# pjmikkol/bwtc

Measured on AMD Instinct MI355X. Metric: MB/s compressed (BWT+encode) on 256 MiB block, higher is better.
Workload: dtype u8/u32/u64 integer

## Files before the change

### bwtc_amd/csrc/bwt_engine.hip

```cpp
#include "bwt_engine.hpp"
#include "radix_sort.hpp"
#include <algorithm>
#include <cmath>
#include <cstdlib>
#include <cstring>
#include <chrono>
#include <ctime>
#include <sys/prctl.h>

namespace bwtc_hip {

constexpr int kLoadTPB = 256;
constexpr int kLoadTile = kLoadTPB * 16;
constexpr u32 kTextPad = 128;

__global__ __launch_bounds__(kLoadTPB) void k_load_hist(const u8* __restrict__ src,
                                                        u8* __restrict__ T, u32 ncopy,
                                                        u32 padded, int reverse, int aligned,
                                                        u32* __restrict__ freqs) {
  __shared__ __attribute__((aligned(16))) u8 s_src[kLoadTile + 48];
  __shared__ u32 s_hist[256 * 16];
  const u32 tid = threadIdx.x;
  for (u32 i = tid; i < 256 * 16; i += kLoadTPB) s_hist[i] = 0;
  const u32 ntiles = (padded + (u32)kLoadTile - 1u) / (u32)kLoadTile;
// ... 462 lines not shown
      else { const u64 full = (fc << need) | ((x_hi << 32) | x_lo); k_lo = full & 0xFFFFFFFFull; k_hi = full >> 32; }
      const u64 ea = ((u64)s_ends[wi] << 32) | (u64)s_ends[wi + 1u];
      const u64 eb = ((u64)s_ends[wi + 2u] << 32) | (u64)s_ends[wi + 3u];
      const u64 etop = off ? (ea << off) | (eb >> (64u - off)) : ea;
      u32 k = 1u;
      if (need <= 64u) k += need ? (u32)__popcll(etop >> (64u - need)) : 0u;
      else k += (u32)__popcll(etop) + (u32)__popcll((off ? (eb << off) : eb) >> (128u - need));
      const u32 i = i_base + t;
      u64 key = k_hi;
      key |= (u64)(i ? (u32)s_c[(int)t - 1] : 0u) << ck.chr_shift;
      key |= (u64)code_level_of(k) << ck.lvl_shift;
      s_key[cntw - 1u - t] = key;
      s_w[cntw - 1u - t] = (u32)k_lo;
    }
  }
  __syncthreads();
  for (u32 j = threadIdx.x; j < cntw; j += 256u) {
    u64 key = s_key[j];
    if (idx_hi) key |= (u64)((n - 1u - (J0 + j)) >> 16) << ck.hi_shift;
    keys[J0 + j] = key;
    const u32 w = s_w[j];
    wout[J0 + j] = w;
    if (plane) plane[J0 + j] = (u8)w;
  }
}

constexpr int kRrTPB = 256;
constexpr int kRrWaves = kRrTPB / kWave;
constexpr int kRrE = 8;
constexpr int kRrChunk = kWave * kRrE;
constexpr int kRrTile = kRrTPB * kRrE;

__device__ __forceinline__ u64 shfl_up1(u64 v) {
  return (u64)__shfl_up((unsigned long long)v, 1, kWave);
}
__device__ __forceinline__ u32 shfl_up1(u32 v) { return __shfl_up(v, 1, kWave); }
__device__ __forceinline__ u64 shfl_down1(u64 v) {
  return (u64)__shfl_down((unsigned long long)v, 1, kWave);
}
__device__ __forceinline__ u32 shfl_down1(u32 v) { return __shfl_down(v, 1, kWave); }

template <typename K, bool INIT>
struct RrMasks {
  u64 head[kRrE], act[kRrE], valid[kRrE];
  u32 sfx[kRrE];
  u32 chr[kRrE];
// ... 1074 lines not shown
  a.off_US = take(lcap * 4);
  a.off_UR = take(lcap * 4);
  a.off_pairs = take((u64)kPairReplicas * 65536 * 4);
  a.off_codes = take((u64)kCodeRows * 256 * 4);
  a.off_runK = take(cap * 4);
  const u64 run_tiles = (cap + kRunTile - 1) / kRunTile + 1;
  a.off_runF = take(run_tiles * 4);
  a.off_runB = take(run_tiles * 4);
  a.total = o;
  return a;
}

static u64 arena_items(u32 max_block) { return std::max<u64>((u64)max_block + 1, 1u << 20); }

u64 BwtEngine::workspace_bytes(u32 max_block) { return plan_arena(arena_items(max_block)).total; }

int BwtEngine::init(int dev, u32 max_block_size) {
  device = dev;
  max_block = max_block_size;
  cap = arena_items(max_block_size);
  std::memset(&stats, 0, sizeof stats);
  BWTC_HIP_TRY(hipSetDevice(dev));
  BWTC_HIP_TRY(hipStreamCreateWithFlags(&stream, hipStreamNonBlocking));
  const ArenaPlan a = plan_arena(cap);
  arena_bytes = a.total;
  BWTC_HIP_TRY(hipMalloc(&arena, arena_bytes));
  u8* base = static_cast<u8*>(arena);
  d_T = base + a.off_T;
  d_out = base + a.off_out;
  d_in = base + a.off_in;
  d_SA = reinterpret_cast<u32*>(base + a.off_SA);
  d_rank = reinterpret_cast<u32*>(base + a.off_rank);
  d_R1 = base + a.off_R1;
  d_R2 = base + a.off_R2;
  d_V0 = reinterpret_cast<u32*>(base + a.off_V0);
  d_V1 = reinterpret_cast<u32*>(base + a.off_V1);
  d_G0 = reinterpret_cast<u32*>(base + a.off_G0);
  d_G1 = reinterpret_cast<u32*>(base + a.off_G1);
  d_GRP = reinterpret_cast<u32*>(base + a.off_GRP);
  d_C0 = base + a.off_C0;
  d_C1 = base + a.off_C1;
  d_P0 = base + a.off_P0;
  d_P1 = base + a.off_P1;
  d_W0 = reinterpret_cast<u32*>(base + a.off_W0);
  d_W1 = reinterpret_cast<u32*>(base + a.off_W1);
  d_table = reinterpret_cast<u32*>(base + a.off_table);
// ... 32 lines not shown
    models_side_stream = !(std::getenv("BWTC_HIP_MODELS_STREAM") && std::getenv("BWTC_HIP_MODELS_STREAM")[0] == '0');
    const char* d = std::getenv("BWTC_HIP_WAVELET_DEPTH");
    if (d && std::atoi(d) > 0) max_inflight = (unsigned)std::atoi(d);
    dense_route = !(std::getenv("BWTC_HIP_DENSE") && std::getenv("BWTC_HIP_DENSE")[0] == '0');
    no_emit = std::getenv("BWTC_HIP_NO_EMIT") != nullptr;
    if (std::getenv("BWTC_HIP_WINDOW_BITS") && std::atoi(std::getenv("BWTC_HIP_WINDOW_BITS")) > 0)
      window_bits = std::min(24, std::atoi(std::getenv("BWTC_HIP_WINDOW_BITS")));
    digit_planes = !(std::getenv("BWTC_HIP_PLANES") && std::getenv("BWTC_HIP_PLANES")[0] == '0');
    split_index = !(std::getenv("BWTC_HIP_SPLIT_INDEX") && std::getenv("BWTC_HIP_SPLIT_INDEX")[0] == '0');
    if (const char* gr = std::getenv("BWTC_HIP_GRAMS")) {
      gram_keys = gr[0] != '0';
      gram_count_override = std::atoi(gr);
    }
    long_keys = !(std::getenv("BWTC_HIP_LONG") && std::getenv("BWTC_HIP_LONG")[0] == '0');
    if (std::getenv("BWTC_HIP_LONG_G2")) long_grams_override = std::atoi(std::getenv("BWTC_HIP_LONG_G2"));
    if (std::getenv("BWTC_HIP_FIN_GROUP")) fin_max_group = std::atoi(std::getenv("BWTC_HIP_FIN_GROUP"));
    if (std::getenv("BWTC_HIP_FIN_WINDOW")) fin_window = std::atoi(std::getenv("BWTC_HIP_FIN_WINDOW"));
    fin_shape_fixed = std::getenv("BWTC_HIP_FIN_GROUP") || std::getenv("BWTC_HIP_FIN_WINDOW");
    fin_wide_short = !(std::getenv("BWTC_HIP_FIN_WIDE") && std::getenv("BWTC_HIP_FIN_WIDE")[0] == '0');
    fin_window = fin_window >= 2048 ? 2048 : 1024;
    fin_max_group = fin_max_group >= 1024 ? 1024 : fin_max_group >= 512 ? 512 : 256;
    if (fin_max_group >= fin_window) fin_max_group = fin_window / 2;
    code_keys = !(std::getenv("BWTC_HIP_KEYS") && std::strcmp(std::getenv("BWTC_HIP_KEYS"), "grams") == 0);
    if (std::getenv("BWTC_HIP_CODE_BITS")) code_bits = std::min(72, std::max(40, std::atoi(std::getenv("BWTC_HIP_CODE_BITS"))));
    finisher = !(std::getenv("BWTC_HIP_FINISHER") && std::getenv("BWTC_HIP_FINISHER")[0] == '0');
    gm_partition_lines = std::getenv("BWTC_HIP_GM_PARTITION") && std::strcmp(std::getenv("BWTC_HIP_GM_PARTITION"), "lines") == 0;
    wt_segmented = !(std::getenv("BWTC_HIP_SEG_STEPS") && std::getenv("BWTC_HIP_SEG_STEPS")[0] == '0');
    gram_min_n = kGramMinN;
    if (std::getenv("BWTC_HIP_GRAM_MIN_N")) gram_min_n = (u32)std::max(64, std::atoi(std::getenv("BWTC_HIP_GRAM_MIN_N")));
    if (std::getenv("BWTC_HIP_LONG_E")) long_items_per_thread = std::atoi(std::getenv("BWTC_HIP_LONG_E")) == 6 ? 6 : 8;
    if (std::getenv("BWTC_HIP_FIN_PASSES")) fin_max_passes = std::max(0, std::atoi(std::getenv("BWTC_HIP_FIN_PASSES")));
    if (std::getenv("BWTC_HIP_FIN_WORDS")) fin_words = std::min(4, std::max(2, std::atoi(std::getenv("BWTC_HIP_FIN_WORDS"))));
    if (std::getenv("BWTC_HIP_LONG_DIRECT")) long_direct = std::getenv("BWTC_HIP_LONG_DIRECT")[0] != '0';
    if (std::getenv("BWTC_HIP_FIN_ROUNDS")) fin_rounds = std::min(4, std::max(1, std::atoi(std::getenv("BWTC_HIP_FIN_ROUNDS"))));
    run_ranks = !(std::getenv("BWTC_HIP_RUNS") && std::getenv("BWTC_HIP_RUNS")[0] == '0');
    local_rounds = !(std::getenv("BWTC_HIP_LOCAL_ROUNDS") && std::getenv("BWTC_HIP_LOCAL_ROUNDS")[0] == '0');
    if (std::getenv("BWTC_HIP_FIN_FLOOR")) fin_floor = (u32)std::max(0, std::atoi(std::getenv("BWTC_HIP_FIN_FLOOR")));
    if (std::getenv("BWTC_HIP_TEXT_ROUNDS")) { text_rounds = std::max(0, std::atoi(std::getenv("BWTC_HIP_TEXT_ROUNDS"))); text_rounds_fixed = true; }
    const char* hg = std::getenv("BWTC_HIP_HUGE_MI");
    if (hg && std::atoi(hg) > 0) huge_group_elements = (u64)std::atoi(hg) << 20;
  }
  if (std::getenv("BWTC_HIP_SCAN") && std::strcmp(std::getenv("BWTC_HIP_SCAN"), "chained") == 0) {
    scan_chain.cap_tiles = (u32)(cap / kScanTile + 4096);
    BWTC_HIP_TRY(hipMalloc(reinterpret_cast<void**>(&scan_chain.status), ((u64)scan_chain.cap_tiles + 1) * 8));
    BWTC_HIP_TRY(hipMemset(scan_chain.status, 0, ((u64)scan_chain.cap_tiles + 1) * 8));
    scan_chain.ticket = scan_chain.status + scan_chain.cap_tiles;
// ... 368 lines not shown
    BWTC_APPLY(0, (u32*)nullptr, (u32*)nullptr, rb.v_free);
  }
#undef BWTC_APPLY
#undef BWTC_APPLY_S
  if (m_next == 0) return 0;
  hipLaunchKernelGGL(k_gather_key2, dim3(ceil_div(m_next, 256 * kSimpleE)), dim3(256), 0, st,
                     (const u32*)rb.v_free, (const u32*)d_GRP, (const u32*)d_rank,
                     carry_next ? (const u8*)re.achr_out : (const u8*)nullptr, recA, m_next, n,
                     (u32)(h_next > 0xFFFFFFFFull ? 0xFFFFFFFFu : h_next), b2k, rkeys, (const u8*)d_T);
  const bool timed = n_sort_events + 2 <= kMaxSortEvents;
  if (timed) BWTC_HIP_TRY(hipEventRecord(ev_sort[n_sort_events++], st));
  sort_pairs<u64>(recA, recB, rb.v_free, rb.v_keys, m_next, kbits, &res->ks, &res->vs, true);
  if (timed) BWTC_HIP_TRY(hipEventRecord(ev_sort[n_sort_events++], st));
  stats.sort_pass_items += (u64)m_next * (u64)((kbits + kRadixBits - 1) / kRadixBits);
  stats.alg_bytes += (u64)m_next * (4 + 4 + 4 + 1 + 8 + (rkeys.mode ? 4 + (run_now ? 1 : 0) : 0)) + sort_bytes(m_next, (kbits + kRadixBits - 1) / kRadixBits, 12, 8, digit_planes);
  res->rec_other = res->ks == recA ? recB : recA;
  res->v_other = res->vs == rb.v_free ? rb.v_keys : rb.v_free;
  return 0;
}

static constexpr int kSmallGram = 526;
static constexpr int kSmallFin = 528;
static constexpr int kSmallFinNext = 540;
int BwtEngine::plan_grams(const KeyPlan& plan, u32 n, const u8* d_lut, GramPlan* gp) {
  hipStream_t st = stream;
  gp->G = 0;
  if (!gram_keys || n < gram_min_n) return 0;
  int g = 1;
  u64 U = plan.sigma;
  while (U * plan.sigma <= kGramMaxU && U * plan.sigma <= (u64)cap / 2 && g < 32) { U *= plan.sigma; ++g; }
  if (g < 2) return 0;
  const u32 nwords = ceil_div((u32)U, 64u);
  u8* present = reinterpret_cast<u8*>(d_SA);
  unsigned long long* bits = reinterpret_cast<unsigned long long*>(present + 64ull * nwords);
  uint4* table = reinterpret_cast<uint4*>(d_rank);
  u32 top = 1;
  for (int t = 1; t < g; ++t) top *= plan.sigma;
  stats.alg_bytes += (u64)n + 64ull * nwords * 2;
  BWTC_HIP_TRY(hipMemsetAsync(present, 0, 64ull * nwords, st));
  hipLaunchKernelGGL(k_gram_mark, dim3(std::min<u32>(ceil_div(n, kGramTile), 4096u)), dim3(256), 0, st,
                     (const u8*)d_T, d_lut, n, g, plan.sigma, top, present);
  hipLaunchKernelGGL(k_gram_pack, dim3(ceil_div(nwords, 256u)), dim3(256), 0, st, (const u8*)present, nwords, bits);
  hipLaunchKernelGGL(k_gram_table, dim3(1), dim3(1024), 0, st, (const unsigned long long*)bits, nwords, table,
                     d_small + kSmallGram);
  BWTC_HIP_TRY(hipMemcpyAsync(h_small + kSmallGram, d_small + kSmallGram, 4, hipMemcpyDeviceToHost, st));
  BWTC_HIP_TRY(wait());
// ... 87 lines not shown
    const bool long_ok = long_keys && implied_idx && emit && key_plane && n >= gram_min_n;
    const bool coded = long_ok && code_keys && finisher && !code_failed;
    auto upload_inverse_lut = [&]() -> int {
      u8 inv[256];
      std::memset(inv, 0, sizeof inv);
      for (int c = 255; c >= 0; --c) if (hist[c] && !(c == 0 && lone_sentinel)) inv[plan.lut[c]] = (u8)c;
      std::memcpy(h_small + kSmallInv, inv, 256);
      BWTC_HIP_TRY(hipMemcpyAsync(d_small + kSmallInv, h_small + kSmallInv, 256, hipMemcpyHostToDevice, st));
      return 0;
    };
    int w_bits = 0;
    RrLong lg;
    lg.w = nullptr; lg.wmask = ~0u; lg.hi_shift = 0; lg.chr_shift = 0; lg.chr_mask = 0; lg.lvl_shift = -1; lg.depth = 0;
    int split_now = split;
    if (coded) {
      split_now = (split_index && n <= (1u << 29)) ? 1 : 0;
      key_bits = code_bits - 32;
      w_bits = 32;
      const int hi_bits = split_now ? 13 : 0;
      CodeKey ck;
      ck.codes = d_codes; ck.kbits = code_bits; ck.hi_shift = key_bits; ck.chr_shift = key_bits + hi_bits; ck.lvl_shift = ck.chr_shift + 8;
      rc = upload_inverse_lut();
      if (rc) return rc;
      BWTC_HIP_TRY(hipMemsetAsync(d_pairs, 0, (size_t)kPairReplicas * 65536 * 4, st));
      const u32 sample_tiles = std::min<u32>(ceil_div(n, kPairTile), 512u);
      hipLaunchKernelGGL(k_pair_counts, dim3(sample_tiles), dim3(256), 0, st, (const u8*)d_T, d_lut, n, d_pairs);
      hipLaunchKernelGGL(k_code_build, dim3(kCodeRows), dim3(256), 0, st, (const u32*)d_pairs, plan.sigma, d_codes, d_small + kSmallError);
      hipLaunchKernelGGL(k_make_keys_code, dim3(ceil_div(n, 1024)), dim3(256), 0, st, (const u8*)d_T, d_lut, ka, d_W0, n, key_plane, split_now, ck);
      lg.hi_shift = ck.hi_shift; lg.chr_shift = ck.chr_shift; lg.chr_mask = 0xFFu; lg.lvl_shift = ck.lvl_shift;
      lk.w = d_W0;
      short_len = 0;
      h = 1;
      stats.alg_bytes += (u64)sample_tiles * kPairTile + (u64)kPairReplicas * 65536 * 8;
      if (std::getenv("BWTC_HIP_DEBUG"))
        std::fprintf(stderr, "code keys: %d + %d bits, sigma %u, %u sampled tiles, character code at bit %d, level at bit %d\n",
                     key_bits, w_bits, plan.sigma, sample_tiles, ck.chr_shift, ck.lvl_shift);
    } else if (long_ok && gp.G > 0) {
      const int cb = std::max(1, bit_width_u64(plan.sigma - 1));
      int G2 = std::min(32 / gp.b, (64 - gp.g * gp.G) / gp.g);
      G2 = std::min(G2, long_grams_override > 0 ? long_grams_override : 2);
      const int hi_bits = split ? 13 : 0;
      if (G2 >= 1 && key_bits + hi_bits + cb <= 64) {
        lk.w = d_W0; lk.G2 = G2; lk.hi_shift = key_bits; lk.chr_shift = key_bits + hi_bits; lk.chr_mask = (1u << cb) - 1u;
        rc = upload_inverse_lut();
        if (rc) return rc;
        w_bits = gp.b * lk.G2;
        if (w_bits < kRadixBits) { lk.first_r = w_bits; lk.first_mask = (1u << std::min(kRadixBits, w_bits + key_bits)) - 1u; }
        short_len = (u32)(gp.g * (gp.G + lk.G2));
        h = (u64)short_len;
        hipLaunchKernelGGL(k_make_keys_gram, dim3(ceil_div(n, 1024)), dim3(256), 0, st, d_T, d_lut,
                           (const uint4*)d_rank, ka, (u32*)nullptr, n, gp.g, gp.G, gp.b, plan.sigma, gp.top, key_plane, split, lk);
// ... 589 lines not shown
```

### bwtc_amd/csrc/bwt_engine.hpp

```cpp
#pragma once
#include "common.hpp"
#include "bwtc_hip.h"
#include "radix_sort.hpp"
#include "scan.hpp"
#include "wavelet_host.hpp"
#include "wavelet_pipeline.hpp"
#include <sys/mman.h>
#include <condition_variable>
#include <future>
#include <map>
#include <mutex>
#include <thread>
#include <memory>
#include <utility>
#include <cstdlib>
#include <functional>
#include <vector>

namespace bwtc_hip {

struct RrEmit;
struct RrLong;
struct FinList;
struct FinShallow;
struct FinOutcome { u32 hard = 0, hard_depth = 0xFFFFFFFFu, left = 0, local = 0; };
constexpr u32 kFinRegions = 16;
struct FinRegions { u32 nreg; u32 wfirst[kFinRegions + 1]; u32 ebase[kFinRegions]; u32 ecount[kFinRegions]; };

struct PinnedGauge {
  std::atomic<uint64_t> now{0}, peak{0};
  void add(uint64_t n) {
    const uint64_t v = now.fetch_add(n) + n;
    uint64_t p = peak.load();
    while (p < v && !peak.compare_exchange_weak(p, v)) {}
  }
  void sub(uint64_t n) { now.fetch_sub(n); }
  static PinnedGauge& get() { static PinnedGauge g; return g; }
};

constexpr size_t kLockedHugePage = (size_t)2 << 20;
constexpr size_t kLockedMapFrom = (size_t)32 << 20;
inline size_t lockedMapBytes(size_t n) { return (n + kLockedHugePage - 1) / kLockedHugePage * kLockedHugePage; }
inline void* lockedHostAlloc(size_t n, int* kind) {
  void* q = nullptr;
  if (n >= kLockedMapFrom && !std::getenv("BWTC_HIP_NO_HUGE_PAGES")) {
// ... 290 lines not shown
  struct RankBuffers { void* rec_keys; void* rec_free; u32* v_keys; u32* v_free; u32* aglob; u32* aglob_next; };
  struct RankResult { u32 m, groups; u64* ks; u32* vs; void* rec_other; u32* v_other; bool finish; u32 text_chars; bool carry;
                      bool ran_run; };
  template <typename K, bool INIT>
  int rank_step(const K* ks, const u32* vs, u32 m, u32 n, u32 short_len, K kmask, RankBuffers& rb,
                struct RrEmit re, bool emit, u64 h_next, RankResult* res, u32 split = 0,
                const struct RrLong* lg = nullptr, bool text = false, bool carry_in = true, bool raw_out = false,
                int run_mode = 0);
  bool dense_route = true;
  bool digit_planes = true;
  int window_bits = 16;
  bool split_index = true;
  bool gram_keys = true;
  int gram_count_override = 0;
  struct GramPlan { int g = 0, G = 0, b = 0; u32 top = 0; };
  int plan_grams(const KeyPlan& plan, u32 n, const u8* d_lut, GramPlan* gp);
  bool no_emit = false;
  bool long_keys = true;
  int long_items_per_thread = 8;
  u32 gram_min_n = 1u << 22;
  bool code_failed = false;
  bool code_keys = true;
  int code_bits = 72;
  u32* d_pairs = nullptr;
  u32* d_codes = nullptr;
  u32* d_parkS = nullptr;
  u64* d_parkHP = nullptr;
  u32 parked = 0;
  u32 park_holes = 0;
  u32* d_hardS = nullptr;
  u64* d_hardHP = nullptr;
  unsigned short* d_hardC = nullptr;
  bool ranks_live = false;
  u32 fin_floor = 12;
  bool finisher = true;
  int fin_window = 1024;
  int fin_max_group = 256;
  int fin_words = 2;
  bool fin_shape_fixed = false;
  bool fin_wide_short = true;
  int fin_window_blk = 1024;
  int fin_group_blk = 256;
  bool long_direct = true;
  int fin_rounds = 3;
  int fin_max_passes = 8;
  int text_rounds = 6;
// ... 68 lines not shown
```

### bwtc_amd/csrc/c_abi.hip

```cpp
#include "bwt_engine.hpp"
#include "gpu_lanes.hpp"
#include "huffman_decoder.hpp"
#include "postprocess.hpp"
#include "wavelet_rebuild.hpp"
#include "prepr_host.hpp"
#include <new>
#include "radix_sort.hpp"
#include "bwtc_hip.h"
#include "entropy_host.hpp"
#include "wavelet_host.hpp"
#include "wavelet_gpu_models.hpp"
#include <sched.h>
#include <algorithm>
#include <atomic>
#include <string>
#include <cstring>
#include <new>
#include <thread>
#include <vector>

using namespace bwtc_hip;

struct bwtc_hip_ctx {
  BwtEngine eng;
// ... 1054 lines not shown
}

int bwtc_hip_test_radix_pairs(bwtc_hip_ctx* ctx, void* keys, void* vals, uint64_t n, uint64_t n_holes, int key_bytes, int val_bytes,
                              int bit_lo, int nbits, int values_mode, int planes) {
  if (!ctx || !keys) return -1;
  BwtEngine& e = ctx->eng;
  typedef unsigned short u16v;
  if (key_bytes == 4 && val_bytes == 4) return test_radix_pairs<u32, u32>(e, static_cast<u32*>(keys), static_cast<u32*>(vals), n, n_holes, bit_lo, nbits, values_mode, planes);
  if (key_bytes == 8 && val_bytes == 4) return test_radix_pairs<u64, u32>(e, static_cast<u64*>(keys), static_cast<u32*>(vals), n, n_holes, bit_lo, nbits, values_mode, planes);
  if (key_bytes == 4 && val_bytes == 2) return test_radix_pairs<u32, u16v>(e, static_cast<u32*>(keys), static_cast<u16v*>(vals), n, n_holes, bit_lo, nbits, values_mode, planes);
  if (key_bytes == 8 && val_bytes == 2) return test_radix_pairs<u64, u16v>(e, static_cast<u64*>(keys), static_cast<u16v*>(vals), n, n_holes, bit_lo, nbits, values_mode, planes);
  return -1;
}

int bwtc_hip_test_radix_long(bwtc_hip_ctx* ctx, uint64_t* keys, void* vals, uint32_t* w, uint64_t n, int val_bytes, int items_per_thread,
                             int kbits, int wbits, int direct_w) {
  if (!ctx || !keys || !vals || !w) return -1;
  BwtEngine& e = ctx->eng;
  typedef unsigned short u16v;
  if (val_bytes == 4 && items_per_thread == 6) return test_radix_long<u32, 6>(e, keys, static_cast<u32*>(vals), w, n, kbits, wbits, direct_w != 0);
  if (val_bytes == 2 && items_per_thread == 6) return test_radix_long<u16v, 6>(e, keys, static_cast<u16v*>(vals), w, n, kbits, wbits, direct_w != 0);
  if (val_bytes == 2 && items_per_thread == 8) return test_radix_long<u16v, 8>(e, keys, static_cast<u16v*>(vals), w, n, kbits, wbits, direct_w != 0);
  return -1;
}

int bwtc_hip_test_radix_segmented(bwtc_hip_ctx* ctx, uint32_t* keys, uint64_t n, int bit_lo, const uint32_t* tile_first, uint32_t nseg) {
  if (!ctx || !keys || !tile_first) return -1;
  BwtEngine& e = ctx->eng;
  const u64 tile = (u64)radix_tile<u32>();
  if (n == 0 || n % tile != 0 || n + kSortCanaryBytes > e.cap) return -1;
  if (bit_lo < 0 || bit_lo + 2 * kRadixBits > 32) return -1;
  if (nseg == 0 || (u64)nseg + 1 > e.cap || tile_first[0] != 0 || (u64)tile_first[nseg] != n / tile) return -1;
  for (u32 s = 0; s < nseg; ++s) if (tile_first[s] > tile_first[s + 1]) return -1;
  BWTC_HIP_TRY(hipSetDevice(e.device));
  hipStream_t st = e.stream;
  u32* k0 = static_cast<u32*>(e.d_R1);
  u32* k1 = static_cast<u32*>(e.d_R2);
  std::vector<u8> plane(n);
  for (u64 i = 0; i < n; ++i) plane[i] = (u8)((keys[i] >> bit_lo) & 255u);
  SortCanaries can;
  BWTC_HIP_TRY(hipMemcpyAsync(k0, keys, n * 4, hipMemcpyHostToDevice, st));
  BWTC_HIP_TRY(hipMemcpyAsync(e.d_P0, plane.data(), n, hipMemcpyHostToDevice, st));
  BWTC_HIP_TRY(hipMemcpyAsync(e.d_V0, tile_first, ((u64)nseg + 1) * 4, hipMemcpyHostToDevice, st));
  BWTC_HIP_TRY(can.put(k0, n * 4, st));
  BWTC_HIP_TRY(can.put(k1, n * 4, st));
  BWTC_HIP_TRY(can.put(e.d_P0, n, st));
// ... 218 lines not shown
```

### bwtc_amd/hip.py

```python
import ctypes
import os

import numpy as np

_HERE = os.path.dirname(os.path.abspath(__file__))
LIB_PATH = os.environ.get("BWTC_HIP_LIB") or os.path.join(_HERE, "lib", "libbwtc_hip.so")

_vp = ctypes.c_void_p
_u32 = ctypes.c_uint32
_u64 = ctypes.c_uint64


class BwtcHipError(RuntimeError):
    def __init__(self, msg, code=None):
        super().__init__(msg)
        self.code = code


E_NO_CODE, E_SHAPE, E_PAST_RECORD, E_RUNS, E_CAPACITY, E_LENGTH = -10, -11, -12, -13, -14, -15


class HuffmanDecodeStats(ctypes.Structure):
    _fields_ = [("route", _u32), ("sections", _u32), ("streams", _u32), ("host_syncs", _u32),
                ("retries", _u32), ("max_code_len", _u32), ("runs", _u64), ("tiles", _u64), ("map_entries", _u64),
# ... 140 lines not shown
REJECT_FLAGS, REJECT_COUNT, REJECT_SCAN, REJECT_STATE, REJECT_TEST = 1, 2, 4, 8, 16


class KernelTimers(ctypes.Structure):
    _fields_ = [("scatter_launches", _u64), ("scatter_bytes", _u64), ("scatter_ms", ctypes.c_double)]


EXPORTS = [
    "bwtc_hip_huffman_decode", "bwtc_hip_huffman_decode_device", "bwtc_hip_huffman_decode_stats_get",
    "bwtc_hip_device_count", "bwtc_hip_version", "bwtc_hip_workspace_bytes", "bwtc_hip_create",
    "bwtc_hip_destroy", "bwtc_hip_stream", "bwtc_hip_get_stats", "bwtc_hip_set_profiling",
    "bwtc_hip_get_kernel_timers", "bwtc_hip_copy_probe", "bwtc_hip_test_gpu_lanes", "bwtc_hip_malloc", "bwtc_hip_free", "bwtc_hip_memcpy_to_device",
    "bwtc_hip_memcpy_to_host", "bwtc_hip_host_alloc", "bwtc_hip_host_free",
    "bwtc_hip_memcpy_to_device_async", "bwtc_hip_copy_wait", "bwtc_hip_wavelet_host_clock", "bwtc_hip_wavelet_host_progress", "bwtc_hip_wavelet_latency", "bwtc_hip_wavelet_routes", "bwtc_hip_host_staging_bytes", "bwtc_hip_host_usable_cpus", "bwtc_hip_n_lf", "bwtc_hip_bwt",
    "bwtc_hip_bwt_block", "bwtc_hip_bwt_block_device", "bwtc_hip_inverse_bwt_block",
    "bwtc_hip_inverse_bwt_block_device", "bwtc_hip_compress_bound",
    "bwtc_hip_huffman_encode_device", "bwtc_hip_huffman_encode", "bwtc_hip_transform_and_encode",
    "bwtc_hip_wavelet_section_stats", "bwtc_hip_transform_and_encode_wavelet", "bwtc_hip_wavelet_encode",
    "bwtc_hip_wavelet_encode_device", "bwtc_hip_wavelet_encode_device_begin", "bwtc_hip_wavelet_encode_end",
    "bwtc_hip_wavelet_encode_device_prepare", "bwtc_hip_wavelet_encode_queue",
    "bwtc_hip_wavelet_depth", "bwtc_hip_wavelet_set_depth", "bwtc_hip_numa_node", "bwtc_hip_host_cpu_slice", "bwtc_hip_set_worker_cpus", "bwtc_hip_wavelet_reset", "bwtc_hip_wavelet_start", "bwtc_hip_host_wavelet_sections", "bwtc_hip_host_wavelet_streams", "bwtc_hip_host_wavelet_streams_lanes", "bwtc_hip_host_huffman_lengths", "bwtc_hip_host_huffman_codes", "bwtc_hip_host_serialize_shape",
    "bwtc_hip_host_sections", "bwtc_hip_host_bwtblock_header", "bwtc_hip_synth", "bwtc_hip_suffix_array",
    "bwtc_hip_test_sort_u32", "bwtc_hip_test_sort_u64", "bwtc_hip_test_scan_u32",
    "bwtc_hip_test_radix_pairs", "bwtc_hip_test_radix_long", "bwtc_hip_test_radix_segmented",
    "bwtc_hip_wavelet_depth_needed", "bwtc_hip_grammar_create", "bwtc_hip_grammar_destroy", "bwtc_hip_grammar_rules", "bwtc_hip_grammar_special_symbols",
    "bwtc_hip_grammar_is_special", "bwtc_hip_grammar_write", "bwtc_hip_grammar_read", "bwtc_hip_pair_replace_device",
    "bwtc_hip_test_pair_stats", "bwtc_hip_precompress", "bwtc_hip_host_precompress", "bwtc_hip_postprocess",
    "bwtc_hip_postprocess_device", "bwtc_hip_postprocess_block", "bwtc_hip_postprocess_stats_get",
    "bwtc_hip_host_postprocess_tiles",
    "bwtc_hip_wavelet_decoder_create", "bwtc_hip_wavelet_decoder_destroy", "bwtc_hip_wavelet_decoder_reset",
    "bwtc_hip_wavelet_decode_bwt_host",
    "bwtc_hip_wavelet_decode_counts", "bwtc_hip_wavelet_decoder_forest", "bwtc_hip_wavelet_rebuild", "bwtc_hip_wavelet_rebuild_device",
    "bwtc_hip_host_wavelet_rebuild", "bwtc_hip_wavelet_decode_stats_get",
]

_lib = None


def load():
    global _lib
    if _lib is not None:
        return _lib
    if not os.path.exists(LIB_PATH):
        raise BwtcHipError(
            "%s not found: build it with `make -C bwtc_amd/csrc` (or __graft_entry__.build()); "
            "there is no CPU fallback" % LIB_PATH)
    L = ctypes.CDLL(LIB_PATH)
# ... 108 lines not shown
    L.bwtc_hip_wavelet_decode_counts.argtypes = [_vp, _vp, _u64, _u64, _vp, ctypes.POINTER(_u64)]
    L.bwtc_hip_wavelet_decoder_forest.argtypes = [_vp, ctypes.POINTER(WForest), _vp, ctypes.POINTER(_u32)]
    L.bwtc_hip_wavelet_rebuild.argtypes = [_vp, ctypes.POINTER(WForest), _vp, _u64, ctypes.POINTER(_u64)]
    L.bwtc_hip_wavelet_rebuild_device.argtypes = L.bwtc_hip_wavelet_rebuild.argtypes
    L.bwtc_hip_host_wavelet_rebuild.argtypes = [ctypes.POINTER(WForest), _vp, _u64, ctypes.POINTER(_u64), _u32, ctypes.POINTER(_u64)]
    L.bwtc_hip_wavelet_decode_stats_get.argtypes = [_vp, ctypes.POINTER(WaveletDecodeStats)]
    L.bwtc_hip_host_huffman_lengths.restype = None
    L.bwtc_hip_host_huffman_lengths.argtypes = [_vp, _vp]
    L.bwtc_hip_host_huffman_codes.restype = None
    L.bwtc_hip_host_huffman_codes.argtypes = [_vp, _vp]
    L.bwtc_hip_host_serialize_shape.restype = _u32
    L.bwtc_hip_host_serialize_shape.argtypes = [_vp, _vp, _u32]
    L.bwtc_hip_host_sections.restype = _u32
    L.bwtc_hip_host_sections.argtypes = [_vp, _vp]
    L.bwtc_hip_host_bwtblock_header.restype = _u32
    L.bwtc_hip_host_bwtblock_header.argtypes = [_vp, _u32, _vp, _u32]
    L.bwtc_hip_suffix_array.argtypes = [_vp, _vp, _u32, _vp]
    L.bwtc_hip_test_sort_u32.argtypes = [_vp, _vp, _vp, _u64, ctypes.c_int]
    L.bwtc_hip_test_sort_u64.argtypes = [_vp, _vp, _vp, _u64, ctypes.c_int]
    L.bwtc_hip_test_scan_u32.argtypes = [_vp, _vp, _u64]
    L.bwtc_hip_test_radix_pairs.argtypes = [_vp, _vp, _vp, _u64, _u64] + [ctypes.c_int] * 6
    L.bwtc_hip_test_radix_long.argtypes = [_vp, _vp, _vp, _vp, _u64] + [ctypes.c_int] * 5
    L.bwtc_hip_test_radix_segmented.argtypes = [_vp, _vp, _u64, ctypes.c_int, _vp, _u32]
    _lib = L
    return L


def _check(rc, what):
    if rc != 0:
        raise BwtcHipError("%s failed with code %d" % (what, rc), rc)


def _ptr(a):
    return a.ctypes.data_as(_vp)


class Grammar:

    def __init__(self):
        self.lib = load()
        self.h = self.lib.bwtc_hip_grammar_create()
        if not self.h:
            raise BwtcHipError("bwtc_hip_grammar_create failed")

    def __del__(self):
        if getattr(self, "h", None):
# ... 544 lines not shown
            vals = None
        nbits = 8 * keys.itemsize if nbits is None else nbits
        _check(self.lib.bwtc_hip_test_radix_pairs(self.handle, _ptr(keys), None if vals is None else _ptr(vals), n, n_holes, keys.itemsize,
                                                  vtype.itemsize, bit_lo, nbits, mode, planes), "bwtc_hip_test_radix_pairs")
        return keys[:n], (None if vals is None else vals[:n])

    def test_radix_long(self, keys, w, kbits, wbits, vtype=np.uint32, items_per_thread=6, direct_w=True):
        keys = np.array(keys, dtype=np.uint64, copy=True)
        w = np.array(w, dtype=np.uint32, copy=True)
        assert keys.size == w.size
        vals = np.zeros(max(keys.size, 1), np.dtype(vtype))
        _check(self.lib.bwtc_hip_test_radix_long(self.handle, _ptr(keys), _ptr(vals), _ptr(w), keys.size, vals.itemsize, items_per_thread,
                                                 kbits, wbits, 1 if direct_w else 0), "bwtc_hip_test_radix_long")
        return keys, vals[:keys.size], w

    def test_radix_segmented(self, keys, bit_lo, tile_first):
        keys = np.array(keys, dtype=np.uint32, copy=True)
        tf = np.array(tile_first, dtype=np.uint32, copy=True)
        assert tf.size >= 2
        _check(self.lib.bwtc_hip_test_radix_segmented(self.handle, _ptr(keys), keys.size, bit_lo, _ptr(tf), tf.size - 1),
               "bwtc_hip_test_radix_segmented")
        return keys


def host_cpu_slice(numa_node, rank, ranks):
    L = load()
    buf = np.zeros(4096, np.uint32)
    n = L.bwtc_hip_host_cpu_slice(int(numa_node), int(rank), int(ranks), _ptr(buf), buf.size)
    if n < 0:
        raise BwtcHipError("bwtc_hip_host_cpu_slice failed with code %d" % n)
    return [int(c) for c in buf[:n]]


def host_staging_bytes():
    L = load()
    a, b = ctypes.c_uint64(0), ctypes.c_uint64(0)
    L.bwtc_hip_host_staging_bytes(ctypes.byref(a), ctypes.byref(b))
    return a.value, b.value


def synth_into(kind, seed, out):
    _check(load().bwtc_hip_synth(kind.encode(), seed, out.size, _ptr(out)), "bwtc_hip_synth")
    return out
```

### include/bwtc_hip.h

```cpp
#ifndef BWTC_HIP_H
#define BWTC_HIP_H
#include <stddef.h>
#include <stdint.h>

#ifdef __cplusplus
extern "C" {
#endif

typedef struct bwtc_hip_ctx bwtc_hip_ctx;

typedef struct bwtc_hip_stats {
  uint32_t n;
  uint32_t rounds;
  uint64_t active_sum;
  uint64_t sort_pass_items;
  float    ms_total;
  float    ms_sort;
  uint32_t route;
  uint32_t finisher_entries;
  uint64_t alg_bytes;
} bwtc_hip_stats;

typedef struct bwtc_hip_kernel_timers {
  uint64_t scatter_launches;
// ... 161 lines not shown
                                  const uint8_t* run_sym, const uint32_t* run_start,
                                  const uint32_t* run_freqs, const uint32_t* dist_offset,
                                  const uint32_t* dist_len, const uint32_t* dist_cnt,
                                  uint32_t threads, char coder, uint32_t* state, uint8_t* out,
                                  uint64_t out_cap, uint64_t* out_bytes);

void     bwtc_hip_host_huffman_lengths(const uint64_t* freqs, uint8_t* clen);
void     bwtc_hip_host_huffman_codes(const uint8_t* clen, uint32_t* code);
uint32_t bwtc_hip_host_serialize_shape(const uint8_t* clen, uint8_t* out, uint32_t cap);
uint32_t bwtc_hip_host_sections(const uint32_t* freqs, uint32_t* section_len);
uint32_t bwtc_hip_host_bwtblock_header(const uint32_t* lf, uint32_t n_lf, uint8_t* out, uint32_t cap);

int bwtc_hip_synth(char kind, uint64_t seed, uint64_t size, uint8_t* out);

int bwtc_hip_suffix_array(bwtc_hip_ctx* ctx, const uint8_t* T, uint32_t length, uint32_t* sa);

int bwtc_hip_test_sort_u32(bwtc_hip_ctx* ctx, uint32_t* keys, uint32_t* vals, uint64_t n, int nbits);
int bwtc_hip_test_sort_u64(bwtc_hip_ctx* ctx, uint64_t* keys, uint32_t* vals, uint64_t n, int nbits);
int bwtc_hip_test_scan_u32(bwtc_hip_ctx* ctx, uint32_t* data, uint64_t n);
int bwtc_hip_test_radix_pairs(bwtc_hip_ctx* ctx, void* keys, void* vals, uint64_t n, uint64_t n_holes, int key_bytes, int val_bytes,
                              int bit_lo, int nbits, int values_mode, int planes);
int bwtc_hip_test_radix_long(bwtc_hip_ctx* ctx, uint64_t* keys, void* vals, uint32_t* w, uint64_t n, int val_bytes, int items_per_thread,
                             int kbits, int wbits, int direct_w);
int bwtc_hip_test_radix_segmented(bwtc_hip_ctx* ctx, uint32_t* keys, uint64_t n, int bit_lo, const uint32_t* tile_first, uint32_t nseg);
int bwtc_hip_test_gpu_lanes(bwtc_hip_ctx* ctx, const uint16_t* w, uint64_t n, const uint64_t* bounds, uint32_t k, int mode,
                            uint8_t* out, uint64_t out_cap, uint64_t* offsets);

typedef struct bwtc_hip_grammar bwtc_hip_grammar;
bwtc_hip_grammar* bwtc_hip_grammar_create(void);
void     bwtc_hip_grammar_destroy(bwtc_hip_grammar* g);
uint32_t bwtc_hip_grammar_rules(const bwtc_hip_grammar* g);
uint32_t bwtc_hip_grammar_special_symbols(const bwtc_hip_grammar* g);
int      bwtc_hip_grammar_is_special(const bwtc_hip_grammar* g, unsigned symbol);
int      bwtc_hip_grammar_write(const bwtc_hip_grammar* g, uint8_t* out, uint64_t cap, uint64_t* bytes);
int      bwtc_hip_grammar_read(bwtc_hip_grammar* g, const uint8_t* in, uint64_t n, uint64_t* consumed);
int      bwtc_hip_pair_replace_device(bwtc_hip_ctx* ctx, bwtc_hip_grammar* g, const uint8_t* d_src, uint64_t n,
                                      uint8_t* d_dst, uint64_t* n_out, uint32_t* replaced);
int      bwtc_hip_test_pair_stats(bwtc_hip_ctx* ctx, const uint8_t* d_src, uint64_t n, uint32_t* pair_cnt, uint32_t* byte_cnt);
int      bwtc_hip_precompress(bwtc_hip_ctx* ctx, bwtc_hip_grammar* g, const char* options, uint8_t* block, uint64_t n,
                              uint64_t* n_out);
int      bwtc_hip_host_precompress(bwtc_hip_grammar* g, const char* options, uint8_t* block, uint64_t n, uint64_t* n_out);
int      bwtc_hip_postprocess(const bwtc_hip_grammar* g, const uint8_t* data, uint64_t n, uint8_t* out, uint64_t cap,
                              uint64_t* n_out);
int      bwtc_hip_postprocess_device(bwtc_hip_ctx* ctx, const bwtc_hip_grammar* g, const uint8_t* d_data, uint64_t n,
                                     uint8_t* d_out, uint64_t cap, uint64_t* n_out);
int      bwtc_hip_postprocess_block(bwtc_hip_ctx* ctx, const bwtc_hip_grammar* g, const uint8_t* data, uint64_t n,
// ... 106 lines not shown
```

Before: 6743.

## Make code keys with persistent range kernel that double-buffers tile staging

Adds a persistent key-making kernel that gives each workgroup a contiguous range of 1024-symbol tiles (about six workgroups per CU). It prefetches the next tile's text into registers and overlaps staging and code-table lookups with key emission, double-buffering the shared code buffer. Bit-plane buffers are cleared incrementally instead of being reinitialised per launch. This is meant to amortise per-tile setup and hide global-load latency. The cost is lower parallelism and more shared memory per workgroup. The old per-tile kernel stays selectable by environment variable, and a test entry point is added.

```diff
diff --git a/bwtc_amd/csrc/bwt_engine.hip b/bwtc_amd/csrc/bwt_engine.hip
--- a/bwtc_amd/csrc/bwt_engine.hip
+++ b/bwtc_amd/csrc/bwt_engine.hip
@@ -508,6 +508,190 @@
     const u32 w = s_w[j];
     wout[J0 + j] = w;
     if (plane) plane[J0 + j] = (u8)w;
+  }
+}
+
+struct KeyTile { u32 J0, cntw, i_base, pre, span; };
+__device__ __forceinline__ KeyTile key_tile(u32 tile, u32 n) {
+  KeyTile t;
+  t.J0 = tile * 1024u;
+  t.cntw = min(1024u, n - t.J0);
+  t.i_base = n - t.J0 - t.cntw;
+  t.pre = t.i_base > 0 ? 1u : 0u;
+  t.span = t.cntw + kCodeLA + 2u;
+  return t;
+}
+__device__ __forceinline__ void stage_codes_load(const u8* __restrict__ T, u32 i_base, u32 count, u32 (&w)[2]) {
+  const u32 a0 = i_base & ~3u, nw = (i_base - a0 + count + 3u) / 4u;
+#pragma unroll
+  for (int e = 0; e < 2; ++e) {
+    const u32 x = threadIdx.x + 256u * e;
+    w[e] = x < nw ? *reinterpret_cast<const u32*>(T + a0 + 4u * x) : 0u;
+  }
+}
+__device__ __forceinline__ void stage_codes_store(const u8* s_lut, u8* s_code, u32 i_base, u32 count, const u32 (&w)[2]) {
+  const u32 nw = ((i_base & 3u) + count + 3u) / 4u;
+#pragma unroll
+  for (int e = 0; e < 2; ++e) {
+    const u32 x = threadIdx.x + 256u * e;
+    if (x < nw)
+      reinterpret_cast<u32*>(s_code)[x] = (u32)s_lut[w[e] & 255u] | ((u32)s_lut[(w[e] >> 8) & 255u] << 8) |
+                                          ((u32)s_lut[(w[e] >> 16) & 255u] << 16) | ((u32)s_lut[w[e] >> 24] << 24);
+  }
+}
+__device__ __forceinline__ void code_lookups(const u32* __restrict__ codes, const u8* s_c, u32 span, u32 (&cw)[5]) {
+  const u32 t0 = 1u + 5u * threadIdx.x;
+#pragma unroll
+  for (u32 e = 0; e < 5u; ++e) {
+    const u32 t = t0 + e;
+    cw[e] = t < span ? codes[(u32)s_c[t - 1u] * 256u + (u32)s_c[t]] : 0u;
+  }
+}
+constexpr u32 kKeyWgPerCu = 6;
+__global__ __launch_bounds__(256) void k_make_keys_code_range(const u8* __restrict__ T, const u8* __restrict__ lut,
+                                                              u64* __restrict__ keys, u32* __restrict__ wout, u32 n,
+                                                              u8* __restrict__ plane, int idx_hi, CodeKey ck,
+                                                              u32 ntiles, u32 range_tiles) {
+  constexpr u32 kTile = 1024;
+  constexpr u32 kPos = 1280;
+  constexpr u32 kBitWords = (kPos * kCodeMaxLen) / 32 + 8;
+  __shared__ u8 s_lut[256];
+  __shared__ __align__(4) u8 s_code[2][kTile + kCodeLA + 24];
+  __shared__ u32 s_c0[256];
+  __shared__ __align__(8) unsigned short s_bp[kPos + 8];
+  __shared__ u32 s_bits[kBitWords];
+  __shared__ u32 s_ends[kBitWords];
+  __shared__ u64 s_key[kTile];
+  __shared__ u32 s_w[kTile];
+  __shared__ u32 scr[256 / kWave];
+  const u32 tid = threadIdx.x, lane = lane_id(), wave = tid / kWave;
+  const u32 slot = (blockIdx.x & 7u) * (gridDim.x >> 3) + (blockIdx.x >> 3);
+  const u32 first = slot * range_tiles;
+  if (first >= ntiles) return;
+  const u32 last = min(first + range_tiles, ntiles);
+  s_lut[tid] = lut[tid];
+  s_c0[tid] = ck.codes[kCodeOrder0 * 256u + tid];
+  for (u32 i = tid; i < kBitWords; i += 256u) { s_bits[i] = 0u; s_ends[i] = 0u; }
+  KeyTile tl = key_tile(first, n), tn = tl;
+  u32 tw[2];
+  stage_codes_load(T, tl.i_base - tl.pre, tl.span + tl.pre, tw);
+  __syncthreads();
+  stage_codes_store(s_lut, s_code[0], tl.i_base - tl.pre, tl.span + tl.pre, tw);
+  bool more = first + 1u < last;
+  if (more) { tn = key_tile(first + 1u, n); stage_codes_load(T, tn.i_base - tn.pre, tn.span + tn.pre, tw); }
+  __syncthreads();
+  u32 cw[5], cwn[5] = {0u, 0u, 0u, 0u, 0u};
+  code_lookups(ck.codes, s_code[0] + ((tl.i_base - tl.pre) & 3u) + tl.pre, tl.span, cw);
+  u32 buf = 0;
+  for (u32 tile = first; tile < last; ++tile) {
+    const u8* s_c = s_code[buf] + ((tl.i_base - tl.pre) & 3u) + tl.pre;
+    u32 lsum = 0;
+#pragma unroll
+    for (u32 e = 0; e < 5u; ++e) lsum += cw[e] >> 27;
+    const u32 incl = wave_scan_add(lsum, lane);
+    if (lane == kWave - 1) scr[wave] = incl;
+    __syncthreads();
+    u32 bp = incl - lsum, total = 0;
+#pragma unroll
+    for (u32 v = 0; v < 256u / kWave; ++v) {
+      const u32 s = scr[v];
+      if (v < wave) bp += s;
+      total += s;
+    }
+    {
+      u32 word = bp >> 5, fill = bp & 31u;
+      u64 acc = 0, eacc = 0;
+#pragma unroll
+      for (u32 e = 0; e < 5u; ++e) {
+        const u32 len = cw[e] >> 27, code = cw[e] & 0x7FFFFFFu;
+        s_bp[5u * tid + e] = (unsigned short)bp;
+        if (len) {
+          acc |= (u64)code << (64u - fill - len);
+          eacc |= 1ull << (64u - fill - len);
+          fill += len;
+          bp += len;
+          if (fill >= 32u) {
+            if ((u32)(acc >> 32)) atomicOr(&s_bits[word], (u32)(acc >> 32));
+            if ((u32)(eacc >> 32)) atomicOr(&s_ends[word], (u32)(eacc >> 32));
+            acc <<= 32; eacc <<= 32;
+            ++word; fill -= 32u;
+          }
+        }
+      }
+      if ((u32)(acc >> 32)) atomicOr(&s_bits[word], (u32)(acc >> 32));
+      if ((u32)(eacc >> 32)) atomicOr(&s_ends[word], (u32)(eacc >> 32));
+    }
+    if (more) stage_codes_store(s_lut, s_code[buf ^ 1u], tn.i_base - tn.pre, tn.span + tn.pre, tw);
+    __syncthreads();
+    KeyTile t2 = tn;
+    const bool more2 = tile + 2u < last;
+    if (more2) { t2 = key_tile(tile + 2u, n); stage_codes_load(T, t2.i_base - t2.pre, t2.span + t2.pre, tw); }
+    if (more) code_lookups(ck.codes, s_code[buf ^ 1u] + ((tn.i_base - tn.pre) & 3u) + tn.pre, tn.span, cwn);
+    const u32 cntw = tl.cntw;
+    const u32 o = 4u * tid;
+    if (o < cntw) {
+      const u32 cnt = min(4u, cntw - o);
+      const uint2 q = *reinterpret_cast<const uint2*>(&s_bp[o]);
+      const u32 st[4] = {q.x & 0xFFFFu, q.x >> 16, q.y & 0xFFFFu, q.y >> 16};
+      const u32 w0 = st[0] >> 5;
+      u32 B[6], E[6];
+#pragma unroll
+      for (u32 v = 0; v < 6u; ++v) { B[v] = s_bits[w0 + v]; E[v] = s_ends[w0 + v]; }
+      u32 prev = (tl.i_base + o) ? (u32)s_c[(int)o - 1] : 0u;
+      u32 d = st[0] & 31u;
+#pragma unroll
+      for (u32 s = 0; s < 4u; ++s) {
+        if (s < cnt) {
+          const u32 t = o + s;
+#pragma unroll
+          for (u32 v = 0; v < 5u; ++v) { B[v] = __funnelshift_l(B[v + 1u], B[v], d); E[v] = __funnelshift_l(E[v + 1u], E[v], d); }
+          B[5] <<= d; E[5] <<= d;
+          const u32 chr = s_c[t];
+          const u32 first_cw = s_c0[chr];
+          const u32 l0 = first_cw >> 27;
+          const u32 need = (u32)ck.kbits - l0;
+          const u64 top = ((u64)B[0] << 32) | (u64)B[1];
+          const u64 etop = ((u64)E[0] << 32) | (u64)E[1];
+          u64 x_hi, x_lo;
+          u32 k = 1u;
+          if (need <= 64u) {
+            const u64 x = top >> (64u - need);
+            x_hi = x >> 32; x_lo = x & 0xFFFFFFFFull;
+            k += (u32)__popcll(etop >> (64u - need));
+          } else {
+            const u32 extra = need - 64u;
+            x_lo = ((top << extra) | (u64)(B[2] >> (32u - extra))) & 0xFFFFFFFFull;
+            x_hi = top >> (32u - extra);
+            k += (u32)__popcll(etop) + (u32)__popc(E[2] >> (32u - extra));
+          }
+          const u64 fc = (u64)(first_cw & 0x7FFFFFFu);
+          u64 k_hi, k_lo;
+          if (need >= 32u) { k_lo = x_lo; k_hi = x_hi | (fc << (need - 32u)); }
+          else { const u64 full = (fc << need) | ((x_hi << 32) | x_lo); k_lo = full & 0xFFFFFFFFull; k_hi = full >> 32; }
+          u64 key = k_hi;
+          key |= (u64)prev << ck.chr_shift;
+          key |= (u64)code_level_of(k) << ck.lvl_shift;
+          s_key[cntw - 1u - t] = key;
+          s_w[cntw - 1u - t] = (u32)k_lo;
+          prev = chr;
+          d = st[(s + 1u) & 3u] - st[s];
+        }
+      }
+    }
+    __syncthreads();
+    for (u32 j = tid; j < cntw; j += 256u) {
+      u64 key = s_key[j];
+      if (idx_hi) key |= (u64)((n - 1u - (tl.J0 + j)) >> 16) << ck.hi_shift;
+      keys[tl.J0 + j] = key;
+      const u32 w = s_w[j];
+      wout[tl.J0 + j] = w;
+      if (plane) plane[tl.J0 + j] = (u8)w;
+    }
+    const u32 nclr = min(kBitWords, (total >> 5) + 2u);
+    for (u32 i = tid; i < nclr; i += 256u) { s_bits[i] = 0u; s_ends[i] = 0u; }
+#pragma unroll
+    for (u32 e = 0; e < 5u; ++e) cw[e] = cwn[e];
+    tl = tn; tn = t2; more = more2; buf ^= 1u;
   }
 }
 
@@ -1628,6 +1812,11 @@
   std::memset(&stats, 0, sizeof stats);
   BWTC_HIP_TRY(hipSetDevice(dev));
   BWTC_HIP_TRY(hipStreamCreateWithFlags(&stream, hipStreamNonBlocking));
+  {
+    int cus = 0;
+    BWTC_HIP_TRY(hipDeviceGetAttribute(&cus, hipDeviceAttributeMultiprocessorCount, dev));
+    cu_count = (u32)std::max(1, cus);
+  }
   const ArenaPlan a = plan_arena(cap);
   arena_bytes = a.total;
   BWTC_HIP_TRY(hipMalloc(&arena, arena_bytes));
@@ -1706,6 +1895,8 @@
     fin_max_group = fin_max_group >= 1024 ? 1024 : fin_max_group >= 512 ? 512 : 256;
     if (fin_max_group >= fin_window) fin_max_group = fin_window / 2;
     code_keys = !(std::getenv("BWTC_HIP_KEYS") && std::strcmp(std::getenv("BWTC_HIP_KEYS"), "grams") == 0);
+    keymaker_tile = std::getenv("BWTC_HIP_KEYMAKER") && std::strcmp(std::getenv("BWTC_HIP_KEYMAKER"), "tile") == 0;
+    if (std::getenv("BWTC_HIP_KEYMAKER_GRID")) keymaker_grid = (u32)std::min(1 << 16, std::max(0, std::atoi(std::getenv("BWTC_HIP_KEYMAKER_GRID"))));
     if (std::getenv("BWTC_HIP_CODE_BITS")) code_bits = std::min(72, std::max(40, std::atoi(std::getenv("BWTC_HIP_CODE_BITS"))));
     finisher = !(std::getenv("BWTC_HIP_FINISHER") && std::getenv("BWTC_HIP_FINISHER")[0] == '0');
     gm_partition_lines = std::getenv("BWTC_HIP_GM_PARTITION") && std::strcmp(std::getenv("BWTC_HIP_GM_PARTITION"), "lines") == 0;
@@ -2120,6 +2311,60 @@
 static constexpr int kSmallGram = 526;
 static constexpr int kSmallFin = 528;
 static constexpr int kSmallFinNext = 540;
+u32 BwtEngine::make_code_keys(u32 n, const u8* d_lut, u32 sigma, u64* keys, u32* w, u8* plane, int split_now, const CodeKey& ck,
+                              const u32* table) {
+  hipStream_t st = stream;
+  note_error(hipMemsetAsync(d_pairs, 0, (size_t)kPairReplicas * 65536 * 4, st));
+  const u32 sample_tiles = std::min<u32>(ceil_div(n, kPairTile), 512u);
+  hipLaunchKernelGGL(k_pair_counts, dim3(sample_tiles), dim3(256), 0, st, (const u8*)d_T, d_lut, n, d_pairs);
+  hipLaunchKernelGGL(k_code_build, dim3(kCodeRows), dim3(256), 0, st, (const u32*)d_pairs, sigma, d_codes, d_small + kSmallError);
+  if (table) note_error(hipMemcpyAsync(d_codes, table, (size_t)kCodeRows * 256 * 4, hipMemcpyHostToDevice, st));
+  const u32 ntiles = ceil_div(n, 1024);
+  if (keymaker_tile) {
+    hipLaunchKernelGGL(k_make_keys_code, dim3(ntiles), dim3(256), 0, st, (const u8*)d_T, d_lut, keys, w, n, plane, split_now, ck);
+    return 1u;
+  }
+  const u32 want = keymaker_grid ? keymaker_grid : std::max(1u, cu_count) * kKeyWgPerCu;
+  const u32 grid = std::max(8u, (std::min(want, ntiles) + 7u) & ~7u);
+  const u32 range_tiles = ceil_div(ntiles, grid);
+  hipLaunchKernelGGL(k_make_keys_code_range, dim3(grid), dim3(256), 0, st, (const u8*)d_T, d_lut, keys, w, n, plane, split_now, ck,
+                     ntiles, range_tiles);
+  return range_tiles;
+}
+
+int BwtEngine::test_code_keys(const u8* d_src, u32 size, int kbits, const u32* table, u64* keys, u32* w, u8* plane, u32* range_tiles) {
+  const u32 n = size + 1u;
+  if ((u64)n > cap || kbits < 40 || kbits > 72) return -1;
+  BWTC_HIP_TRY(hipSetDevice(device));
+  hipStream_t st = stream;
+  u32 hist_T[256];
+  int rc = load_text(d_src, size, n, true, hist_T);
+  if (rc) return rc;
+  const KeyPlan plan = plan_keys(hist_T, n, h_small[kSmallFreqs] == 0, true);
+  std::memcpy(h_small + kSmallLut, plan.lut, 256);
+  BWTC_HIP_TRY(hipMemcpyAsync(d_small + kSmallLut, h_small + kSmallLut, 256, hipMemcpyHostToDevice, st));
+  const int split_now = (split_index && n <= (1u << 29)) ? 1 : 0;
+  const int key_bits = kbits - 32, hi_bits = split_now ? 13 : 0;
+  CodeKey ck;
+  ck.codes = d_codes; ck.kbits = kbits; ck.hi_shift = key_bits; ck.chr_shift = key_bits + hi_bits; ck.lvl_shift = ck.chr_shift + 8;
+  u64* ka = static_cast<u64*>(d_R1);
+  const u32 rt = make_code_keys(n, reinterpret_cast<const u8*>(d_small + kSmallLut), plan.sigma, ka, d_W0, d_P0, split_now, ck, table);
+  if (range_tiles) *range_tiles = rt;
+  BWTC_HIP_TRY(hipMemcpyAsync(h_small + kSmallError, d_small + kSmallError, 4, hipMemcpyDeviceToHost, st));
+  BWTC_HIP_TRY(hipMemcpyAsync(keys, ka, (size_t)n * 8, hipMemcpyDeviceToHost, st));
+  BWTC_HIP_TRY(hipMemcpyAsync(w, d_W0, (size_t)n * 4, hipMemcpyDeviceToHost, st));
+  BWTC_HIP_TRY(hipMemcpyAsync(plane, d_P0, n, hipMemcpyDeviceToHost, st));
+  BWTC_HIP_TRY(wait());
+  BWTC_HIP_TRY(hipGetLastError());
+  BWTC_HIP_TRY(take_sticky_error());
+  if (h_small[kSmallError] & 2u) {
+    BWTC_HIP_TRY(hipMemsetAsync(d_small + kSmallError, 0, 4, st));
+    BWTC_HIP_TRY(wait());
+    return 1;
+  }
+  return 0;
+}
+
 int BwtEngine::plan_grams(const KeyPlan& plan, u32 n, const u8* d_lut, GramPlan* gp) {
   hipStream_t st = stream;
   gp->G = 0;
@@ -2253,11 +2498,8 @@
       ck.codes = d_codes; ck.kbits = code_bits; ck.hi_shift = key_bits; ck.chr_shift = key_bits + hi_bits; ck.lvl_shift = ck.chr_shift + 8;
       rc = upload_inverse_lut();
       if (rc) return rc;
-      BWTC_HIP_TRY(hipMemsetAsync(d_pairs, 0, (size_t)kPairReplicas * 65536 * 4, st));
       const u32 sample_tiles = std::min<u32>(ceil_div(n, kPairTile), 512u);
-      hipLaunchKernelGGL(k_pair_counts, dim3(sample_tiles), dim3(256), 0, st, (const u8*)d_T, d_lut, n, d_pairs);
-      hipLaunchKernelGGL(k_code_build, dim3(kCodeRows), dim3(256), 0, st, (const u32*)d_pairs, plan.sigma, d_codes, d_small + kSmallError);
-      hipLaunchKernelGGL(k_make_keys_code, dim3(ceil_div(n, 1024)), dim3(256), 0, st, (const u8*)d_T, d_lut, ka, d_W0, n, key_plane, split_now, ck);
+      (void)make_code_keys(n, d_lut, plan.sigma, ka, d_W0, key_plane, split_now, ck);
       lg.hi_shift = ck.hi_shift; lg.chr_shift = ck.chr_shift; lg.chr_mask = 0xFFu; lg.lvl_shift = ck.lvl_shift;
       lk.w = d_W0;
       short_len = 0;
diff --git a/bwtc_amd/csrc/bwt_engine.hpp b/bwtc_amd/csrc/bwt_engine.hpp
--- a/bwtc_amd/csrc/bwt_engine.hpp
+++ b/bwtc_amd/csrc/bwt_engine.hpp
@@ -21,6 +21,7 @@
 
 struct RrEmit;
 struct RrLong;
+struct CodeKey;
 struct FinList;
 struct FinShallow;
 struct FinOutcome { u32 hard = 0, hard_depth = 0xFFFFFFFFu, left = 0, local = 0; };
@@ -357,6 +358,11 @@
   bool code_failed = false;
   bool code_keys = true;
   int code_bits = 72;
+  bool keymaker_tile = false;
+  u32 keymaker_grid = 0;
+  u32 cu_count = 0;
+  u32 make_code_keys(u32 n, const u8* d_lut, u32 sigma, u64* keys, u32* w, u8* plane, int split_now, const CodeKey& ck, const u32* table = nullptr);
+  int test_code_keys(const u8* d_src, u32 size, int kbits, const u32* table, u64* keys, u32* w, u8* plane, u32* range_tiles);
   u32* d_pairs = nullptr;
   u32* d_codes = nullptr;
   u32* d_parkS = nullptr;
diff --git a/bwtc_amd/csrc/c_abi.hip b/bwtc_amd/csrc/c_abi.hip
--- a/bwtc_amd/csrc/c_abi.hip
+++ b/bwtc_amd/csrc/c_abi.hip
@@ -1100,6 +1100,19 @@
   if (val_bytes == 2 && items_per_thread == 6) return test_radix_long<u16v, 6>(e, keys, static_cast<u16v*>(vals), w, n, kbits, wbits, direct_w != 0);
   if (val_bytes == 2 && items_per_thread == 8) return test_radix_long<u16v, 8>(e, keys, static_cast<u16v*>(vals), w, n, kbits, wbits, direct_w != 0);
   return -1;
+}
+
+int bwtc_hip_test_code_keys(bwtc_hip_ctx* ctx, const uint8_t* block, uint32_t size, int kbits, const uint32_t* table, uint64_t* keys,
+                            uint32_t* w, uint8_t* plane, uint32_t* range_tiles) {
+  if (!ctx || (!block && size) || !keys || !w || !plane) return -1;
+  BwtEngine& e = ctx->eng;
+  if (size > e.max_block) return -1;
+  if (table)
+    for (uint32_t i = 0; i < 257u * 256u; ++i) if ((table[i] >> 27) < 1u || (table[i] >> 27) > 26u) return -1;
+  BWTC_HIP_TRY(hipSetDevice(e.device));
+  const int rc = stage_in(e, block, size);
+  if (rc) return rc;
+  return e.test_code_keys(e.d_in, size, kbits, table, keys, w, plane, range_tiles);
 }
 
 int bwtc_hip_test_radix_segmented(bwtc_hip_ctx* ctx, uint32_t* keys, uint64_t n, int bit_lo, const uint32_t* tile_first, uint32_t nseg) {
diff --git a/bwtc_amd/hip.py b/bwtc_amd/hip.py
--- a/bwtc_amd/hip.py
+++ b/bwtc_amd/hip.py
@@ -186,7 +186,7 @@
     "bwtc_hip_wavelet_depth", "bwtc_hip_wavelet_set_depth", "bwtc_hip_numa_node", "bwtc_hip_host_cpu_slice", "bwtc_hip_set_worker_cpus", "bwtc_hip_wavelet_reset", "bwtc_hip_wavelet_start", "bwtc_hip_host_wavelet_sections", "bwtc_hip_host_wavelet_streams", "bwtc_hip_host_wavelet_streams_lanes", "bwtc_hip_host_huffman_lengths", "bwtc_hip_host_huffman_codes", "bwtc_hip_host_serialize_shape",
     "bwtc_hip_host_sections", "bwtc_hip_host_bwtblock_header", "bwtc_hip_synth", "bwtc_hip_suffix_array",
     "bwtc_hip_test_sort_u32", "bwtc_hip_test_sort_u64", "bwtc_hip_test_scan_u32",
-    "bwtc_hip_test_radix_pairs", "bwtc_hip_test_radix_long", "bwtc_hip_test_radix_segmented",
+    "bwtc_hip_test_radix_pairs", "bwtc_hip_test_radix_long", "bwtc_hip_test_radix_segmented", "bwtc_hip_test_code_keys",
     "bwtc_hip_wavelet_depth_needed", "bwtc_hip_grammar_create", "bwtc_hip_grammar_destroy", "bwtc_hip_grammar_rules", "bwtc_hip_grammar_special_symbols",
     "bwtc_hip_grammar_is_special", "bwtc_hip_grammar_write", "bwtc_hip_grammar_read", "bwtc_hip_pair_replace_device",
     "bwtc_hip_test_pair_stats", "bwtc_hip_precompress", "bwtc_hip_host_precompress", "bwtc_hip_postprocess",
@@ -341,6 +341,7 @@
     L.bwtc_hip_test_radix_pairs.argtypes = [_vp, _vp, _vp, _u64, _u64] + [ctypes.c_int] * 6
     L.bwtc_hip_test_radix_long.argtypes = [_vp, _vp, _vp, _vp, _u64] + [ctypes.c_int] * 5
     L.bwtc_hip_test_radix_segmented.argtypes = [_vp, _vp, _u64, ctypes.c_int, _vp, _u32]
+    L.bwtc_hip_test_code_keys.argtypes = [_vp, _vp, _u32, ctypes.c_int, _vp, _vp, _vp, _vp, _vp]
     _lib = L
     return L
 
@@ -931,6 +932,18 @@
                "bwtc_hip_test_radix_segmented")
         return keys
 
+    def test_code_keys(self, data, kbits=72, table=None):
+        data = np.ascontiguousarray(data, dtype=np.uint8)
+        if table is not None:
+            table = np.ascontiguousarray(table, dtype=np.uint32)
+            assert table.size == 257 * 256
+        n = data.size + 1
+        keys, w, plane = np.zeros(n, np.uint64), np.zeros(n, np.uint32), np.zeros(n, np.uint8)
+        rt = _u32(0)
+        _check(self.lib.bwtc_hip_test_code_keys(self.handle, _ptr(data) if data.size else None, data.size, kbits, None if table is None else _ptr(table), _ptr(keys), _ptr(w),
+                                                _ptr(plane), ctypes.byref(rt)), "bwtc_hip_test_code_keys")
+        return keys, w, plane, int(rt.value)
+
 
 def host_cpu_slice(numa_node, rank, ranks):
     L = load()
diff --git a/include/bwtc_hip.h b/include/bwtc_hip.h
--- a/include/bwtc_hip.h
+++ b/include/bwtc_hip.h
@@ -207,6 +207,8 @@
                               int bit_lo, int nbits, int values_mode, int planes);
 int bwtc_hip_test_radix_long(bwtc_hip_ctx* ctx, uint64_t* keys, void* vals, uint32_t* w, uint64_t n, int val_bytes, int items_per_thread,
                              int kbits, int wbits, int direct_w);
+int bwtc_hip_test_code_keys(bwtc_hip_ctx* ctx, const uint8_t* block, uint32_t size, int kbits, const uint32_t* table, uint64_t* keys,
+                            uint32_t* w, uint8_t* plane, uint32_t* range_tiles);
 int bwtc_hip_test_radix_segmented(bwtc_hip_ctx* ctx, uint32_t* keys, uint64_t n, int bit_lo, const uint32_t* tile_first, uint32_t nseg);
 int bwtc_hip_test_gpu_lanes(bwtc_hip_ctx* ctx, const uint16_t* w, uint64_t n, const uint64_t* bounds, uint32_t k, int mode,
                             uint8_t* out, uint64_t out_cap, uint64_t* offsets);
```

Result: slower. 6526 (-3.2%).
